# WangHelin1997/SSR-Speech

Measured on AMD Instinct MI355X. Metric: codec-tokens/sec/GPU (AR decode) + RTF for 10 s TTS, English 830M, higher is better.
Workload: dtype f32; 1 GPU; English-830M-shape zero-shot TTS decode, cfg_stride=5, top_k=40/top_p=0.8 sampling, batch=1 (2 CFG rows) per GPU; L=130 phonemes, 160-frame prompt (demo/5895_34622_000026_000002.wav, first 3.2 s, wmencodec codes), context 304..324; utterances_per_gpu=1, rows=2, graph=True, steps_completed=25, pair_launches=True

## Files before the change

ssr-speech_amd/csrc/gemv.hip:

```cpp
#include <stdlib.h>
#include "common.h"

namespace {

struct GemvK {
  ssrhip_gemv_args a;
  int nslice;
  int slice_len;
  int nch;
  int groups_x;
  int hd;
  int seg_shift;
  int rows_max;
  long long* prof;
  int rows_per, rows_rem;
};


long long* g_gemv_prof = nullptr;
constexpr int PRO_LN_REGS = 3;
constexpr int MAXCH = 8;
constexpr int MAX_IT = 8;

constexpr int NJ = 4;
// ... 699 lines not shown
  for (int j = 0; j < NUW; ++j) {
    float4 (&wj)[4] = w[j % DEPTH];
    float acc[B][2];
#pragma unroll
    for (int b = 0; b < B; ++b) acc[b][0] = acc[b][1] = 0.f;
#pragma unroll
    for (int i = 0; i < 4; ++i) {
#pragma unroll
      for (int b = 0; b < B; ++b) acc[b][i & 1] = dot4(wj[i], xr[b][i], acc[b][i & 1]);
      if (j + DEPTH < NUW) {
        __builtin_amdgcn_sched_barrier(0);
        wj[i] = ld_nt(Wg + (size_t)((wave + SEG_NW * (j + DEPTH)) >> sh) * K + i * 256);
        __builtin_amdgcn_sched_barrier(0);
      }
    }
    float mine = 0.f;
#pragma unroll
    for (int b = 0; b < B; ++b) {
      const float sum = wave_sum(acc[b][0] + acc[b][1]);
      if (lane == b) mine = sum;
    }
    if (lane < B) part[(wave + SEG_NW * j) * B + lane] = mine;
  }
  __syncthreads();
  if (t < nrows * B) {
    float v = 0.f;
    for (int s2 = 0; s2 < S; ++s2) v += part[(rfin * S + s2) * B + bfin];
    finalize(p, g, nfin, bfin, v, efin, kvb);
  }
}

constexpr int PAIR_D = 2048, PAIR_NE = 4, PAIR_TH = SEG_TH + 64 * PAIR_NE, PAIR_GRAN = 2 * PAIR_D, PAIR_PF = 3, PAIR_DEPTH = 4, PAIR_NUWA = 8;
constexpr int PAIR_SPINS = 4000000;
constexpr long long PAIR_WAIT_TICKS = 100000000;
struct PairK {
  GemvK a, b;
  unsigned long long* gran;
  unsigned long long* gran_next;
  int* gave_up;
};
typedef float pair_v4f __attribute__((ext_vector_type(4)));
__device__ __forceinline__ void pair_sweep8(const unsigned long long* p, pair_v4f (&g)[8]) {
  asm volatile(
      "global_load_dwordx4 %0, %8, off sc1\n\tglobal_load_dwordx4 %1, %8, off offset:1024 sc1\n\t"
      "global_load_dwordx4 %2, %8, off offset:2048 sc1\n\tglobal_load_dwordx4 %3, %8, off offset:3072 sc1\n\t"
      "global_load_dwordx4 %4, %9, off sc1\n\tglobal_load_dwordx4 %5, %9, off offset:1024 sc1\n\t"
      "global_load_dwordx4 %6, %9, off offset:2048 sc1\n\tglobal_load_dwordx4 %7, %9, off offset:3072 sc1\n\t"
      "s_waitcnt vmcnt(0)"
      : "=&v"(g[0]), "=&v"(g[1]), "=&v"(g[2]), "=&v"(g[3]), "=&v"(g[4]), "=&v"(g[5]), "=&v"(g[6]), "=&v"(g[7])
      : "v"(p), "v"(p + 512)
      : "memory");
}

template <int NUWB, int EARLY = 0, int PFX = PAIR_PF>
__device__ __forceinline__ void pair_stream_b(const PairK& p, int t, int lane, int wave, float4 (&xr)[2][4], float4 (&w)[PAIR_DEPTH][4],
                                              const RowEpi& efinB, float* partB, float* aux, const float* xs, const size_t* kvoff) {
  constexpr int B = 2, DEPTH = PAIR_DEPTH, PF = PFX, SB = 2, SHB = 1, RB = NUWB * SEG_NW / SB;
  static_assert(PFX >= EARLY && PFX <= PAIR_DEPTH, "units requested at (1b) start behind the early ones and fit the ring");
  static_assert(EARLY == 0 || EARLY == 2, "ring slots 2 and 3 are the ones the merge form's A phase leaves free");
  const ssrhip_gemv_args& bb = p.b.a;
  const int rB0 = (int)blockIdx.x * RB, segB = wave & (SB - 1);
  const int bfin = t % B, rfinB = min(t / B, RB - 1), nfinB = rB0 + rfinB;
  const float* WgB = bb.W + (size_t)rB0 * bb.K + segB * SEG + lane * 4;
  __syncthreads();
#pragma unroll
  for (int j = EARLY; j < PF; ++j)
#pragma unroll
    for (int i = 0; i < 4; ++i) w[(j + EARLY) % DEPTH][i] = ld_nt(WgB + (size_t)((wave + SEG_NW * j) >> SHB) * bb.K + i * 256);
  __syncthreads();
#pragma unroll
  for (int b = 0; b < B; ++b)
#pragma unroll
    for (int i = 0; i < 4; ++i) xr[b][i] = *reinterpret_cast<const float4*>(xs + b * PAIR_D + segB * SEG + (i * 64 + lane) * 4);
#pragma unroll
  for (int j = PF; j < DEPTH; ++j)
#pragma unroll
    for (int i = 0; i < 4; ++i) w[(j + EARLY) % DEPTH][i] = ld_nt(WgB + (size_t)((wave + SEG_NW * j) >> SHB) * bb.K + i * 256);
  {
    float m[B], q[B];
#pragma unroll
    for (int b = 0; b < B; ++b) {
      float s0 = 0.f;
#pragma unroll
      for (int i = 0; i < 4; ++i) s0 += (xr[b][i].x + xr[b][i].y) + (xr[b][i].z + xr[b][i].w);
      m[b] = wave_sum(s0) * (1.0f / SEG);
      float q0 = 0.f;
#pragma unroll
      for (int i = 0; i < 4; ++i) {
        const float dx = xr[b][i].x - m[b], dy = xr[b][i].y - m[b], dz = xr[b][i].z - m[b], dw = xr[b][i].w - m[b];
        q0 += (dx * dx + dy * dy) + (dz * dz + dw * dw);
      }
      q[b] = wave_sum(q0);
      if (wave < SB && lane == 0) { aux[(wave * B + b) * 2] = m[b]; aux[(wave * B + b) * 2 + 1] = q[b]; }
    }
    __syncthreads();
#pragma unroll
    for (int b = 0; b < B; ++b) {
      float mean = 0.f, M2 = 0.f, dev = 0.f;
      for (int s2 = 0; s2 < SB; ++s2) mean += aux[(s2 * B + b) * 2];
      mean /= (float)SB;
      for (int s2 = 0; s2 < SB; ++s2) { const float dm = aux[(s2 * B + b) * 2] - mean; M2 += aux[(s2 * B + b) * 2 + 1]; dev = fmaf(dm, dm, dev); }
      const float var = (M2 + (float)SEG * dev) / (float)bb.K;
      const float rstd = 1.0f / sqrtf(var + bb.ln_eps);
#pragma unroll
      for (int i = 0; i < 4; ++i)
        xr[b][i] = make_float4((xr[b][i].x - mean) * rstd, (xr[b][i].y - mean) * rstd, (xr[b][i].z - mean) * rstd, (xr[b][i].w - mean) * rstd);
    }
  }
#pragma unroll
  for (int j = 0; j < NUWB; ++j) {
    float4 (&wj)[4] = w[(j + EARLY) % DEPTH];
    float acc[B][2];
#pragma unroll
    for (int b = 0; b < B; ++b) acc[b][0] = acc[b][1] = 0.f;
#pragma unroll
    for (int i = 0; i < 4; ++i) {
#pragma unroll
      for (int b = 0; b < B; ++b) acc[b][i & 1] = dot4(wj[i], xr[b][i], acc[b][i & 1]);
      if (j + DEPTH < NUWB) {
        __builtin_amdgcn_sched_barrier(0);
        wj[i] = ld_nt(WgB + (size_t)((wave + SEG_NW * (j + DEPTH)) >> SHB) * bb.K + i * 256);
        __builtin_amdgcn_sched_barrier(0);
      }
    }
    float mine = 0.f;
#pragma unroll
    for (int b = 0; b < B; ++b) {
      const float sum = wave_sum(acc[b][0] + acc[b][1]);
      if (lane == b) mine = sum;
    }
    if (lane < B) partB[(wave + SEG_NW * j) * B + lane] = mine;
  }
  __syncthreads();
  if (t < RB * B) {
    float v = 0.f;
    for (int s2 = 0; s2 < SB; ++s2) v += partB[(rfinB * SB + s2) * B + bfin];
    float* kvb[2] = {bb.kv.pool + kvoff[bfin * 2], bb.kv.pool + kvoff[bfin * 2 + 1]};
    finalize(p.b, 0, nfinB, bfin, v, efinB, kvb);
  }
}

template <int SA, int NPRE>
__device__ __forceinline__ void pair_edge_role(const PairK& p, int e, int lane, const float* partA, float* xs, size_t* kvoff) {
  constexpr int B = 2, RA = 8;
  const ssrhip_gemv_args& a = p.a.a;
  const ssrhip_gemv_args& bb = p.b.a;
  const int rA0 = (int)blockIdx.x * RA;
  RowEpi efinA = {0.f, 0.f};
  if (e == 0 && lane < RA * B) {
    efinA.bias = a.bias ? a.bias[rA0 + (lane >> 1)] : 0.f;
    efinA.resid = a.y[(size_t)(lane & 1) * a.y_stride + rA0 + (lane >> 1)];
    p.gran_next[(size_t)blockIdx.x * (RA * B) + lane] = 0ull;
  }
  if (bb.epi == SSRHIP_EPI_QKV_APPEND && e == 1 && lane < B) {
    const int pos = bb.kv_pos[lane];
    const int page = bb.kv.table[(size_t)lane * bb.kv.max_pages + (pos / SSRHIP_PAGE)];
    const size_t k0 = ((((size_t)page * bb.kv.n_layer + bb.layer) * 2 + 0) * bb.kv.n_head) * SSRHIP_PAGE + (pos % SSRHIP_PAGE);
    const size_t v0 = ((((size_t)page * bb.kv.n_layer + bb.layer) * 2 + 1) * bb.kv.n_head) * SSRHIP_PAGE + (pos % SSRHIP_PAGE);
    kvoff[lane * 2 + 0] = k0 * bb.kv.head_dim;
    kvoff[lane * 2 + 1] = v0 * bb.kv.head_dim;
  }
#pragma unroll
  for (int i = 0; i < NPRE; ++i) __syncthreads();
  __syncthreads();
  if (e == 0 && lane < RA * B) {
    const int r = lane >> 1, b = lane & 1, n = rA0 + r;
    float v = 0.f;
    for (int s2 = 0; s2 < SA; ++s2) v += partA[(r * SA + s2) * B + b];
    v += efinA.bias;
    const float out = efinA.resid + v;
    a.y[(size_t)b * a.y_stride + n] = out;
    const unsigned long long gval = ((unsigned long long)1u << 32) | (unsigned long long)__float_as_uint(out);
    __hip_atomic_store(p.gran + (size_t)n * 2 + b, gval, __ATOMIC_RELAXED, __HIP_MEMORY_SCOPE_AGENT);
  }
  __syncthreads();
  pair_v4f g[8];
  bool done = false;
  const int max_spins = (*p.gave_up != 0) ? 64 : PAIR_SPINS;
  const long long t_begin = wall_clock64();
  for (int spin = 0; spin < max_spins && !done; ++spin) {
    bool all = true;
    pair_sweep8(p.gran + (size_t)e * 1024 + lane * 2, g);
#pragma unroll
    for (int i = 0; i < 8; ++i) {
      all = all && (__float_as_uint(g[i][1]) == 1u) && (__float_as_uint(g[i][3]) == 1u);
      const int gi = e * 1024 + (i >> 2) * 512 + (i & 3) * 128 + lane * 2;
      xs[(gi >> 1)] = g[i][0];
      xs[PAIR_D + (gi >> 1)] = g[i][2];
    }
    done = __all(all);
    if (!done) {
      __builtin_amdgcn_s_sleep(2);
// ... 32 lines not shown
    float4 w[DEPTH][4];
#pragma unroll
    for (int j = 0; j < DEPTH; ++j)
#pragma unroll
      for (int i = 0; i < 4; ++i) w[j][i] = ld_nt(WgA + (size_t)((wave + SEG_NW * j) >> SHA) * a.K + i * 256);
#pragma unroll
    for (int j = 0; j < NUWA; ++j) {
      float4 (&wj)[4] = w[j % DEPTH];
      float acc[B][2];
#pragma unroll
      for (int b = 0; b < B; ++b) acc[b][0] = acc[b][1] = 0.f;
#pragma unroll
      for (int i = 0; i < 4; ++i) {
#pragma unroll
        for (int b = 0; b < B; ++b) acc[b][i & 1] = dot4(wj[i], xr[b][i], acc[b][i & 1]);
        if (j + DEPTH < NUWA) {
          __builtin_amdgcn_sched_barrier(0);
          wj[i] = ld_nt(WgA + (size_t)((wave + SEG_NW * (j + DEPTH)) >> SHA) * a.K + i * 256);
          __builtin_amdgcn_sched_barrier(0);
        }
      }
      float mine = 0.f;
#pragma unroll
      for (int b = 0; b < B; ++b) {
        const float sum = wave_sum(acc[b][0] + acc[b][1]);
        if (lane == b) mine = sum;
      }
      if (lane < B) partA[(wave + SEG_NW * j) * B + lane] = mine;
    }
    __syncthreads();
    pair_stream_b<NUWB>(p, t, lane, wave, xr, w, efinB, partB, aux, xs, kvoff);
  } else {
    pair_edge_role<SA, 0>(p, wave - SEG_NW, lane, partA, xs, kvoff);
  }
}

template <int NUWB, int EARLY = 0, int PFX = PAIR_PF>
__global__ __launch_bounds__(PAIR_TH, 2) void gemv_pair_merge_kernel(const PairK p) {
  constexpr int B = 2, DEPTH = PAIR_DEPTH, SEG_CS = SegCS<B>::v;
  constexpr int RA = 8, SA = 2, SHA = 1;
  constexpr int RB = NUWB * SEG_NW / 2;
  extern __shared__ __attribute__((aligned(16))) float wtab[];
  __shared__ float partA[RA * SA * B];
  __shared__ float partB[RB * 2 * B];
  __shared__ float aux[2 * B * 2];
  __shared__ __attribute__((aligned(16))) float xs[B * PAIR_D];
  __shared__ size_t kvoff[B * 2];
  const ssrhip_gemv_args& a = p.a.a;
  const ssrhip_gemv_args& bb = p.b.a;
  const int t = threadIdx.x, lane = t & 63, wave = __builtin_amdgcn_readfirstlane(t >> 6);
  if (wave >= SEG_NW) {
    pair_edge_role<SA, 2>(p, wave - SEG_NW, lane, partA, xs, kvoff);
  } else {
    const int K = a.K, rA0 = (int)blockIdx.x * RA, seg = wave & (SA - 1);
    const float* WgA = a.W + (size_t)rA0 * K + seg * SEG + lane * 4;
    RowEpi efinB = {0.f, 0.f};
    efinB.bias = bb.bias ? bb.bias[(int)blockIdx.x * RB + min(t / B, RB - 1)] : 0.f;
    const int hd = p.a.hd, H = K / hd, MS = a.max_splits;
    float4 co[B][SEG_CS];
    float2 cml[SEG_CS];
    int ns[B];
#pragma unroll
    for (int b = 0; b < B; ++b) ns[b] = (a.row_len[b] + SSRHIP_PAGE - 1) / SSRHIP_PAGE;
    {
      const int tt = t % (B * H);
      const float* ml = a.part_ml + (size_t)tt * MS * 2;
#pragma unroll
      for (int i = 0; i < SEG_CS; ++i) cml[i] = *reinterpret_cast<const float2*>(ml + 2 * min(i, MS - 1));
      const int e = t * 4, h = e / hd, d = e % hd;
#pragma unroll
      for (int b = 0; b < B; ++b) {
        const float* po = a.part_o + (((size_t)b * H + h) * MS) * hd + d;
#pragma unroll
        for (int s2 = 0; s2 < SEG_CS; ++s2) co[b][s2] = ld4(po + (size_t)min(s2, MS - 1) * hd);
      }
    }
    float4 w[DEPTH][4];
#pragma unroll
    for (int j = 0; j < 2; ++j)
#pragma unroll
      for (int i = 0; i < 4; ++i) w[j][i] = ld_nt(WgA + (size_t)((wave + SEG_NW * j) >> SHA) * K + i * 256);
    if constexpr (EARLY == 2) {
      const float* WgB = bb.W + (size_t)((int)blockIdx.x * RB) * bb.K + (wave & 1) * SEG + lane * 4;
#pragma unroll
      for (int j = 0; j < 2; ++j)
#pragma unroll
        for (int i = 0; i < 4; ++i) w[2 + j][i] = ld_nt(WgB + (size_t)((wave + SEG_NW * j) >> 1) * bb.K + i * 256);
    }
    {
      const int tt = t % (B * H);
      const bool keep = t < B * H;
      const int n = ns[tt / H];
      const float* ml = a.part_ml + (size_t)tt * MS * 2;
      float M = -INFINITY;
#pragma unroll
      for (int i = 0; i < SEG_CS; ++i)
        if (i < n) M = fmaxf(M, cml[i].x);
      for (int s2 = SEG_CS; s2 < n; ++s2) M = fmaxf(M, ld2_late(ml + 2 * s2).x);
      float den = 0.f;
#pragma unroll
      for (int i = 0; i < SEG_CS; ++i)
        if (i < n) den = fmaf(expf(cml[i].x - M), cml[i].y, den);
      for (int s2 = SEG_CS; s2 < n; ++s2) { const float2 v = ld2_late(ml + 2 * s2); den = fmaf(expf(v.x - M), v.y, den); }
      const float inv = 1.0f / den;
#pragma unroll
      for (int i = 0; i < SEG_CS; ++i)
        if (keep && i < n) wtab[tt * MS + i] = expf(cml[i].x - M) * inv;
      for (int s2 = SEG_CS; s2 < n; ++s2) { const float wv = expf(ld2_late(ml + 2 * s2).x - M) * inv; if (keep) wtab[tt * MS + s2] = wv; }
    }
    __syncthreads();
    {
      const int e = t * 4, h = e / hd, d = e % hd;
#pragma unroll
      for (int b = 0; b < B; ++b) {
        const float* wt = wtab + (b * H + h) * MS;
        float4 acc = make_float4(0.f, 0.f, 0.f, 0.f);
#pragma unroll
        for (int s2 = 0; s2 < SEG_CS; ++s2) {
          const bool in = s2 < ns[b];
          const float ws = in ? wt[s2] : 0.f;
          acc.x = fmaf(ws, in ? co[b][s2].x : 0.f, acc.x);
          acc.y = fmaf(ws, in ? co[b][s2].y : 0.f, acc.y);
          acc.z = fmaf(ws, in ? co[b][s2].z : 0.f, acc.z);
          acc.w = fmaf(ws, in ? co[b][s2].w : 0.f, acc.w);
        }
        const float* po = a.part_o + (((size_t)b * H + h) * MS) * hd + d;
        for (int s2 = SEG_CS; s2 < ns[b]; ++s2) {
          const float ws = wt[s2];
          const float4 o = ld4_late(po + (size_t)s2 * hd);
          acc.x = fmaf(ws, o.x, acc.x);
          acc.y = fmaf(ws, o.y, acc.y);
          acc.z = fmaf(ws, o.z, acc.z);
          acc.w = fmaf(ws, o.w, acc.w);
        }
        *reinterpret_cast<float4*>(xs + b * K + e) = acc;
      }
    }
    __syncthreads();
    float4 xr[B][4];
#pragma unroll
    for (int b = 0; b < B; ++b)
#pragma unroll
      for (int i = 0; i < 4; ++i) xr[b][i] = *reinterpret_cast<const float4*>(xs + b * K + seg * SEG + (i * 64 + lane) * 4);
#pragma unroll
    for (int j = 0; j < 2; ++j) {
      float acc[B][2];
#pragma unroll
      for (int b = 0; b < B; ++b) acc[b][0] = acc[b][1] = 0.f;
#pragma unroll
      for (int i = 0; i < 4; ++i)
#pragma unroll
        for (int b = 0; b < B; ++b) acc[b][i & 1] = dot4(w[j][i], xr[b][i], acc[b][i & 1]);
      float mine = 0.f;
#pragma unroll
      for (int b = 0; b < B; ++b) {
        const float sum = wave_sum(acc[b][0] + acc[b][1]);
        if (lane == b) mine = sum;
      }
      if (lane < B) partA[(wave + SEG_NW * j) * B + lane] = mine;
    }
    __syncthreads();
    pair_stream_b<NUWB, EARLY, PFX>(p, t, lane, wave, xr, w, efinB, partB, aux, xs, kvoff);
  }
}

int g_seg_mode = -1;

template <int B>
bool try_seg(const ssrhip_gemv_args* a, int num_cu, hipStream_t s) {
  if (a->K % SEG != 0) return false;
  const int S = a->K / SEG;
  if (S != 1 && S != 2 && S != 4 && S != 8) return false;
  if (a->pro == SSRHIP_PRO_LAYERNORM && a->ln_w != nullptr) return false;
  const int H = a->kv.head_dim > 0 ? a->K / a->kv.head_dim : 0;
  if (a->pro == SSRHIP_PRO_ATTN_COMBINE && (a->K != 2048 || a->max_splits < 1 || a->groups != 1 || B * H > SEG_TH || a->kv.head_dim % 4 != 0)) return false;
  int G = (2 * num_cu) / a->groups;
  if (a->pro == SSRHIP_PRO_ATTN_COMBINE && !getenv("SSRHIP_GEMV_SEG_COMBINE_2")) G = num_cu;
  if (G > a->N) G = a->N;
  if (G < 1) G = 1;
  const int rows_max = (a->N + G - 1) / G;
  if (rows_max * B > SEG_TH) return false;
  GemvK p;
  p.a = *a;
  p.nslice = S;
  p.slice_len = SEG;
  p.nch = 4;
  p.seg_shift = (S == 1) ? 0 : (S == 2) ? 1 : (S == 4) ? 2 : 3;
  p.rows_max = rows_max;
  p.rows_per = a->N / G;
  p.rows_rem = a->N % G;
  p.prof = g_gemv_prof;
  p.groups_x = G;
  p.hd = (a->kv.head_dim > 0) ? a->kv.head_dim : 1;
  size_t smem = (size_t)rows_max * S * B * sizeof(float);
  if (a->pro == SSRHIP_PRO_LAYERNORM) smem += (size_t)S * B * 2 * sizeof(float);
  if (a->pro == SSRHIP_PRO_ATTN_COMBINE) smem += ((size_t)B * a->K + (size_t)B * H * a->max_splits) * sizeof(float);
  smem = (smem + 15) / 16 * 16;
  int segu_depth = 4;
  if (const char* e = getenv("SSRHIP_GEMV_SEGU")) { segu_depth = atoi(e); if (segu_depth != 0 && segu_depth != 2) segu_depth = 4; }
  if constexpr (B == 2) {
    const int G1 = num_cu / a->groups;
    if (segu_depth && a->pro != SSRHIP_PRO_ATTN_COMBINE && G1 >= 1 && a->N % G1 == 0 && ((a->N / G1) * S) % SEG_NW == 0) {
      const int nuw = (a->N / G1) * S / SEG_NW;
      if (nuw == 4 || nuw == 6 || nuw == 8) {
        p.rows_max = p.rows_per = a->N / G1;
        p.rows_rem = 0;
        p.groups_x = G1;
        size_t sm = (size_t)p.rows_per * S * B * sizeof(float) + (size_t)S * B * 2 * sizeof(float);
        sm = (sm + 15) / 16 * 16;
        const dim3 g1(G1, a->groups);
#define SEGU_LAUNCH(PRO_, NUW_)                                                                                                       \
        do {                                                                                                                           \
          if (segu_depth == 2) hipLaunchKernelGGL((gemv_segu_kernel<B, PRO_, NUW_, 2>), g1, dim3(SEG_TH), sm, s, p);                    \
          else hipLaunchKernelGGL((gemv_segu_kernel<B, PRO_, NUW_, 4>), g1, dim3(SEG_TH), sm, s, p);                                    \
        } while (0)
        if (a->pro == SSRHIP_PRO_LAYERNORM) {
          if (nuw == 4) SEGU_LAUNCH(SSRHIP_PRO_LAYERNORM, 4); else if (nuw == 6) SEGU_LAUNCH(SSRHIP_PRO_LAYERNORM, 6); else SEGU_LAUNCH(SSRHIP_PRO_LAYERNORM, 8);
        } else {
// ... 14 lines not shown
      if constexpr (B <= 2) { if (two) { hipLaunchKernelGGL((gemv_seg_kernel<B, SSRHIP_PRO_LAYERNORM, true>), grid, dim3(SEG_TH), smem, s, p); break; } }
      hipLaunchKernelGGL((gemv_seg_kernel<B, SSRHIP_PRO_LAYERNORM, false>), grid, dim3(SEG_TH), smem, s, p);
      break;
    case SSRHIP_PRO_ATTN_COMBINE:
      if constexpr (B <= 2) { if (two) { hipLaunchKernelGGL((gemv_seg_kernel<B, SSRHIP_PRO_ATTN_COMBINE, true>), grid, dim3(SEG_TH), smem, s, p); break; } }
      hipLaunchKernelGGL((gemv_seg_kernel<B, SSRHIP_PRO_ATTN_COMBINE, false>), grid, dim3(SEG_TH), smem, s, p);
      break;
    default:
      if constexpr (B <= 2) { if (two) { hipLaunchKernelGGL((gemv_seg_kernel<B, SSRHIP_PRO_NONE, true>), grid, dim3(SEG_TH), smem, s, p); break; } }
      hipLaunchKernelGGL((gemv_seg_kernel<B, SSRHIP_PRO_NONE, false>), grid, dim3(SEG_TH), smem, s, p);
      break;
  }
  return true;
}

int g_num_cu = 0;
int g_blocks_per_cu = 3;

}

int ssrhip_gemv_mfma_launch(const ssrhip_gemv_args* a, hipStream_t s);
int ssrhip_gemv_mfma32_launch(const ssrhip_gemv_args* a, hipStream_t s);

#ifdef SSR_GEMV_PROFILE
extern "C" void ssrhip_debug_gemv_prof(void* dev_ptr) { g_gemv_prof = (long long*)dev_ptr; }
#endif

static thread_local char g_pair_why[200] = "";
const char* ssrhip_gemv_pair_why() { return g_pair_why; }

static const char* pair_device_refusal(int num_cu) {
  static const char* verdict = nullptr;
  static bool asked = false;
  if (asked) return verdict;
  asked = true;
  static char buf[200];
  if (num_cu < 256) { snprintf(buf, sizeof(buf), "the device reports %d CUs (a pair launch needs its 256 workgroups resident together)", num_cu); return verdict = buf; }
  for (const char* name : {"ROC_GLOBAL_CU_MASK", "HSA_CU_MASK", "HSA_CU_MASK_SKIP_INIT"}) {
    const char* e = getenv(name);
    if (e && e[0]) { snprintf(buf, sizeof(buf), "%s is set: fewer CUs than the device reports may be usable", name); return verdict = buf; }
  }
  int nb[4] = {0, 0, 0, 0};
  hipError_t e0 = hipOccupancyMaxActiveBlocksPerMultiprocessor(&nb[0], gemv_pair_kernel<4>, PAIR_TH, 0);
  hipError_t e1 = hipOccupancyMaxActiveBlocksPerMultiprocessor(&nb[1], gemv_pair_kernel<6>, PAIR_TH, 0);
  hipError_t e2 = hipOccupancyMaxActiveBlocksPerMultiprocessor(&nb[2], gemv_pair_kernel<8>, PAIR_TH, 0);
  hipError_t e3 = hipOccupancyMaxActiveBlocksPerMultiprocessor(&nb[3], gemv_pair_merge_kernel<8, 2>, PAIR_TH, 16 * 1024);
  if (e0 != hipSuccess || e1 != hipSuccess || e2 != hipSuccess || e3 != hipSuccess || nb[0] < 1 || nb[1] < 1 || nb[2] < 1 || nb[3] < 1) {
    snprintf(buf, sizeof(buf), "the occupancy calculator places %d / %d / %d / %d workgroups of the pair kernels on a CU (need >= 1 each)", nb[0], nb[1], nb[2], nb[3]);
    return verdict = buf;
  }
  return verdict = nullptr;
}

static int pair_nuwb(const ssrhip_gemv_args* a, const ssrhip_gemv_args* b, int num_cu, bool* merge) {
  *merge = false;
  auto no = [](const char* why) { snprintf(g_pair_why, sizeof(g_pair_why), "%s", why); return 0; };
  int mode = 2;
  if (const char* e = getenv("SSRHIP_GEMV_PAIR")) mode = (e[0] == '0') ? 0 : (e[0] == '1') ? 1 : 2;
  if (mode == 0) return no("SSRHIP_GEMV_PAIR=0");
  if (const char* why = pair_device_refusal(num_cu)) return no(why);
  if (a->B != 2 || b->B != 2 || a->groups != 1 || b->groups != 1) return no("not a 2-row, single-group launch");
  if (a->x_tiled || a->y_tiled || a->w_tiled || b->x_tiled || b->y_tiled || b->w_tiled) return no("tiled layouts");
  if (a->act != SSRHIP_ACT_NONE || a->epi != SSRHIP_EPI_RESIDUAL || a->N != PAIR_D || !a->y || !a->W) return no("the first launch is not a residual GEMV with N = 2048 (the pair kernels are built for d_model 2048)");
  if (a->pro == SSRHIP_PRO_NONE) {
    if (a->K != 8192 || !a->x) return no("FFN2 form needs K = 8192");
  } else if (a->pro == SSRHIP_PRO_ATTN_COMBINE) {
    if (mode < 2) return no("SSRHIP_GEMV_PAIR=1: the merge form is off");
    const int hd = a->kv.head_dim;
    if (a->K != 2048 || !a->part_o || !a->part_ml || !a->row_len || a->max_splits < 1 || hd <= 0 || hd % 4 != 0 || a->K % hd != 0 || 2 * (a->K / hd) > SEG_TH) return no("merge form needs K = 2048 and split-KV partials");
    if ((size_t)2 * (a->K / hd) * a->max_splits * sizeof(float) > 16 * 1024) return no("merge weights exceed 16 KB of LDS (context too long for the merge form)");
    *merge = true;
  } else {
    return no("the first launch has a LayerNorm prologue");
  }
  if (b->pro != SSRHIP_PRO_LAYERNORM || b->ln_w || b->ln_b || b->K != PAIR_D || b->x != a->y || b->x_stride != a->y_stride || !b->W || !b->y) return no("the second launch is not LayerNorm (folded) + Linear on the first one's output");
  if (b->epi != SSRHIP_EPI_STORE && b->epi != SSRHIP_EPI_QKV_APPEND) return no("second launch: epilogue");
  if (b->epi == SSRHIP_EPI_QKV_APPEND && !(b->N == 3 * b->K && b->kv.pool && b->kv.table && b->kv_pos && b->kv.head_dim > 0)) return no("second launch: QKV append without a cache");
  if (b->N % 256 != 0) return no("second launch: N not a multiple of 256");
  const int nuwb = (b->N / 256) * 2 / SEG_NW;
  if ((b->N / 256) * 2 % SEG_NW != 0 || (nuwb != 4 && nuwb != 6 && nuwb != 8)) return no("second launch: N not in {4096, 6144, 8192}");
  if (*merge && nuwb != 8) return no("the merge form is instantiated for FFN1 only");
  g_pair_why[0] = 0;
  return nuwb;
}

static void ensure_num_cu() {
  if (g_num_cu == 0) {
    int dev = 0, cu = 0;
    if (hipGetDevice(&dev) == hipSuccess && hipDeviceGetAttribute(&cu, hipDeviceAttributeMultiprocessorCount, dev) == hipSuccess && cu > 0) g_num_cu = cu;
    else g_num_cu = 256;
    if (const char* e = getenv("SSRHIP_GEMV_BLOCKS_PER_CU")) { const int v = atoi(e); if (v >= 1 && v <= 3) g_blocks_per_cu = v; }
  }
}

extern "C" int ssrhip_pair_buffer(int32_t i, int32_t n) {
  if (n < 2 || i < 0 || i >= n) return -1;
  return (i == n - 1 && n % 3 == 1) ? 1 : i % 3;
}

extern "C" int ssrhip_gemv_pair_applicable(const ssrhip_gemv_args* a, const ssrhip_gemv_args* b) {
  if (!a || !b) return 0;
  ensure_num_cu();
  bool merge;
  return pair_nuwb(a, b, g_num_cu, &merge) != 0;
}

extern "C" int ssrhip_gemv_pair(const ssrhip_gemv_args* a, const ssrhip_gemv_args* b, void* ws, int32_t buf, int32_t buf_next, ssrhip_stream_t stream) {
  SSR_REQUIRE(a && b && ws, "ssrhip_gemv_pair: null argument");
  SSR_REQUIRE(buf >= 0 && buf < 3 && buf_next >= 0 && buf_next < 3 && buf != buf_next, "ssrhip_gemv_pair: granule buffers %d -> %d (0..2, different)", buf, buf_next);
  ensure_num_cu();
  bool merge = false;
  const int nuwb = pair_nuwb(a, b, g_num_cu, &merge);
  if (!nuwb) return 1;
  PairK p;
  auto fill = [](GemvK& k, const ssrhip_gemv_args* g, int S) {
    k.a = *g; k.nslice = S; k.slice_len = SEG; k.nch = 4; k.groups_x = 256; k.hd = (g->kv.head_dim > 0) ? g->kv.head_dim : 1;
    k.seg_shift = (S == 8) ? 3 : 1; k.rows_max = k.rows_per = g->N / 256; k.rows_rem = 0; k.prof = nullptr;
  };
  fill(p.a, a, merge ? 2 : 8);
  fill(p.b, b, 2);
  unsigned long long* gran = (unsigned long long*)ws;
  p.gran = gran + (size_t)buf * PAIR_GRAN;
  p.gran_next = gran + (size_t)buf_next * PAIR_GRAN;
  p.gave_up = (int*)(gran + 3 * (size_t)PAIR_GRAN);
  hipStream_t s = (hipStream_t)stream;
  if (merge) {
    const size_t sm = ((size_t)2 * (a->K / a->kv.head_dim) * a->max_splits * sizeof(float) + 15) / 16 * 16;
    const char* ee = getenv("SSRHIP_GEMV_PAIR_EARLY");
    if (ee && ee[0] == '0') hipLaunchKernelGGL((gemv_pair_merge_kernel<8, 0>), dim3(256), dim3(PAIR_TH), sm, s, p);
    else hipLaunchKernelGGL((gemv_pair_merge_kernel<8, 2>), dim3(256), dim3(PAIR_TH), sm, s, p);
  } else if (nuwb == 4) hipLaunchKernelGGL((gemv_pair_kernel<4>), dim3(256), dim3(PAIR_TH), 0, s, p);
  else if (nuwb == 6) hipLaunchKernelGGL((gemv_pair_kernel<6>), dim3(256), dim3(PAIR_TH), 0, s, p);
  else hipLaunchKernelGGL((gemv_pair_kernel<8>), dim3(256), dim3(PAIR_TH), 0, s, p);
  SSR_LAUNCH_CHECK();
  return 0;
}

extern "C" int ssrhip_gemv_pair_status(const void* ws, ssrhip_stream_t stream) {
  SSR_REQUIRE(ws, "ssrhip_gemv_pair_status: null workspace");
  int flag = 0;
  if (hipStreamSynchronize((hipStream_t)stream) != hipSuccess) { ssrhip_set_error("ssrhip_gemv_pair_status: stream synchronize failed"); return -1; }
  if (hipMemcpy(&flag, (const char*)ws + 3 * (size_t)PAIR_GRAN * 8, sizeof(int), hipMemcpyDeviceToHost) != hipSuccess) {
    ssrhip_set_error("ssrhip_gemv_pair_status: copy failed");
    return -1;
  }
  if (flag) {
    if (hipMemset(const_cast<void*>(ws), 0, SSRHIP_PAIR_WS_BYTES) != hipSuccess) { ssrhip_set_error("ssrhip_gemv_pair_status: re-zeroing the workspace failed"); return -1; }
  }
  return flag ? 1 : 0;
}

extern "C" int ssrhip_gemv(const ssrhip_gemv_args* a, ssrhip_stream_t stream) {
  SSR_REQUIRE(a && a->W && a->y, "ssrhip_gemv: null argument");
  SSR_REQUIRE(a->N > 0 && a->groups >= 1 && a->K > 0, "ssrhip_gemv: bad N/K/groups");
  if (a->B > 16) return ssrhip_gemv_mfma32_launch(a, (hipStream_t)stream);
  if (a->B > 4) return ssrhip_gemv_mfma_launch(a, (hipStream_t)stream);
  SSR_REQUIRE(a->B == 1 || a->B == 2 || a->B == 4, "ssrhip_gemv: B=%d not in {1,2,4} or 5..32", a->B);
  SSR_REQUIRE(!a->x_tiled && !a->y_tiled && !a->w_tiled, "ssrhip_gemv: the tiled activation / weight layouts are for 5..32 rows only");
  SSR_REQUIRE(a->pro != SSRHIP_PRO_ATTN_COMBINE || (a->kv.head_dim > 0 && a->K <= 2048 && a->B * (a->K / a->kv.head_dim) <= 256), "ssrhip_gemv: combine prologue needs K <= 2048 and B*H <= 256");
  SSR_REQUIRE(a->K > 0 && a->K % 4 == 0 && a->K <= 8192, "ssrhip_gemv: K=%d must be a multiple of 4, <= 8192", a->K);
  SSR_REQUIRE(a->N > 0 && a->groups >= 1, "ssrhip_gemv: bad N/groups");
  ensure_num_cu();
  if (a->pro != SSRHIP_PRO_NONE) {
    SSR_REQUIRE(a->groups == 1 || a->pro == SSRHIP_PRO_LAYERNORM, "ssrhip_gemv: combine prologue needs groups==1");
    if (a->pro == SSRHIP_PRO_LAYERNORM) SSR_REQUIRE(a->x && ((a->ln_w && a->ln_b) || (!a->ln_w && !a->ln_b)), "ssrhip_gemv: LayerNorm prologue needs x and either both or none of ln_w/ln_b");
    if (a->pro == SSRHIP_PRO_ATTN_COMBINE) {
      SSR_REQUIRE(a->part_o && a->part_ml && a->row_len && a->kv.head_dim > 0 && a->K % a->kv.head_dim == 0 && a->kv.head_dim % 4 == 0,
                  "ssrhip_gemv: combine prologue needs part_o, part_ml, row_len, kv.head_dim");
    }
  } else {
    SSR_REQUIRE(a->x, "ssrhip_gemv: x is null");
  }
  if (a->epi == SSRHIP_EPI_QKV_APPEND) {
    SSR_REQUIRE(a->N == 3 * a->K && a->groups == 1 && a->kv.pool && a->kv.table && a->kv_pos && a->kv.head_dim > 0,
                "ssrhip_gemv: QKV epilogue needs N==3K and a kv cache");
  }
  if (g_seg_mode < 0) { const char* e = getenv("SSRHIP_GEMV_SEG"); g_seg_mode = (e && e[0] == '0') ? 0 : 1; }
  if (g_seg_mode) {
    bool done = false;
    switch (a->B) {
      case 1: done = try_seg<1>(a, g_num_cu, (hipStream_t)stream); break;
      case 2: done = try_seg<2>(a, g_num_cu, (hipStream_t)stream); break;
// ... 54 lines not shown
```

Measured before the change: 5351 codec-tokens/s.

## Add LDS ring-buffer merge pair kernel with dedicated DMA loader waves

Adds a ring_merge_kernel variant of the merged attention-out plus QKV pair GEMV. Two extra loader waves use global_load_lds to stream second-GEMV weight units into an LDS ring while the compute waves run the first GEMV and the gather waves wait on cross-block granules. This is meant to hide the second GEMV's weight fetch latency behind the grid-wide handoff. It is on by default with a 2-slot ring, so it uses much more LDS and extra waves, which may lower occupancy or make it fall back to the register form when the merge weights do not fit. Optional profiling timestamps and lab variants are compiled out by default.

```diff
diff --git a/ssr-speech_amd/csrc/gemv.hip b/ssr-speech_amd/csrc/gemv.hip
--- a/ssr-speech_amd/csrc/gemv.hip
+++ b/ssr-speech_amd/csrc/gemv.hip
@@ -775,6 +775,11 @@
       : "memory");
 }
 
+#ifdef SSR_GEMV_PROFILE
+#define PSTAMP(i) do { if (p.a.prof && threadIdx.x == 0) p.a.prof[(size_t)blockIdx.x * 8 + (i)] = wall_clock64(); } while (0)
+#else
+#define PSTAMP(i) do { } while (0)
+#endif
 template <int NUWB, int EARLY = 0, int PFX = PAIR_PF>
 __device__ __forceinline__ void pair_stream_b(const PairK& p, int t, int lane, int wave, float4 (&xr)[2][4], float4 (&w)[PAIR_DEPTH][4],
                                               const RowEpi& efinB, float* partB, float* aux, const float* xs, const size_t* kvoff) {
@@ -785,12 +790,15 @@
   const int rB0 = (int)blockIdx.x * RB, segB = wave & (SB - 1);
   const int bfin = t % B, rfinB = min(t / B, RB - 1), nfinB = rB0 + rfinB;
   const float* WgB = bb.W + (size_t)rB0 * bb.K + segB * SEG + lane * 4;
-  __syncthreads();
+  PSTAMP(2);
+  __syncthreads();
+  PSTAMP(3);
 #pragma unroll
   for (int j = EARLY; j < PF; ++j)
 #pragma unroll
     for (int i = 0; i < 4; ++i) w[(j + EARLY) % DEPTH][i] = ld_nt(WgB + (size_t)((wave + SEG_NW * j) >> SHB) * bb.K + i * 256);
   __syncthreads();
+  PSTAMP(4);
 #pragma unroll
   for (int b = 0; b < B; ++b)
 #pragma unroll
@@ -853,7 +861,9 @@
       if (lane == b) mine = sum;
     }
     if (lane < B) partB[(wave + SEG_NW * j) * B + lane] = mine;
-  }
+    if (j == 0) PSTAMP(5);
+  }
+  PSTAMP(6);
   __syncthreads();
   if (t < RB * B) {
     float v = 0.f;
@@ -861,6 +871,7 @@
     float* kvb[2] = {bb.kv.pool + kvoff[bfin * 2], bb.kv.pool + kvoff[bfin * 2 + 1]};
     finalize(p.b, 0, nfinB, bfin, v, efinB, kvb);
   }
+  PSTAMP(7);
 }
 
 template <int SA, int NPRE>
@@ -999,6 +1010,7 @@
   if (wave >= SEG_NW) {
     pair_edge_role<SA, 2>(p, wave - SEG_NW, lane, partA, xs, kvoff);
   } else {
+    PSTAMP(0);
     const int K = a.K, rA0 = (int)blockIdx.x * RA, seg = wave & (SA - 1);
     const float* WgA = a.W + (size_t)rA0 * K + seg * SEG + lane * 4;
     RowEpi efinB = {0.f, 0.f};
@@ -1084,6 +1096,7 @@
       }
     }
     __syncthreads();
+    PSTAMP(1);
     float4 xr[B][4];
 #pragma unroll
     for (int b = 0; b < B; ++b)
@@ -1111,6 +1124,372 @@
   }
 }
 
+constexpr int RING_SLOT = 8192;
+constexpr int RING_FILL = 16;
+typedef __attribute__((address_space(3))) void* ring_lds_ptr_t;
+
+__device__ __forceinline__ void ring_dma_kib(const float* gsrc, unsigned lds_dst) {
+  unsigned keep;
+  asm volatile("s_mov_b32 %0, m0\n\ts_mov_b32 m0, %2\n\ts_nop 0\n\tglobal_load_lds_dwordx4 %1, off nt\n\ts_mov_b32 m0, %0"
+               : "=&s"(keep) : "v"(gsrc), "s"(lds_dst) : "memory");
+}
+template <int N>
+__device__ __forceinline__ void ring_wait_vm() { asm volatile("s_waitcnt vmcnt(%0)" :: "n"(N) : "memory"); }
+
+__device__ __forceinline__ void ring_fill(const float* WgL, int K, unsigned ring_addr, int L, int s) {
+#pragma unroll
+  for (int ww = 0; ww < 4; ++ww) {
+    const int w = 4 * L + ww;
+    const float* src = WgL + (size_t)((w + SEG_NW * (2 + s)) >> 1) * K + (w & 1) * SEG;
+#pragma unroll
+    for (int i = 0; i < 4; ++i) ring_dma_kib(src + i * 256, __builtin_amdgcn_readfirstlane(ring_addr + (unsigned)(s * RING_SLOT + w * 1024 + i * 256) * 4u));
+  }
+}
+
+__device__ __forceinline__ void ring_sweep16(const unsigned long long* p, pair_v4f (&g)[16]) {
+  asm volatile(
+      "global_load_dwordx4 %0, %16, off sc1\n\tglobal_load_dwordx4 %1, %16, off offset:1024 sc1\n\t"
+      "global_load_dwordx4 %2, %16, off offset:2048 sc1\n\tglobal_load_dwordx4 %3, %16, off offset:3072 sc1\n\t"
+      "global_load_dwordx4 %4, %17, off sc1\n\tglobal_load_dwordx4 %5, %17, off offset:1024 sc1\n\t"
+      "global_load_dwordx4 %6, %17, off offset:2048 sc1\n\tglobal_load_dwordx4 %7, %17, off offset:3072 sc1\n\t"
+      "global_load_dwordx4 %8, %18, off sc1\n\tglobal_load_dwordx4 %9, %18, off offset:1024 sc1\n\t"
+      "global_load_dwordx4 %10, %18, off offset:2048 sc1\n\tglobal_load_dwordx4 %11, %18, off offset:3072 sc1\n\t"
+      "global_load_dwordx4 %12, %19, off sc1\n\tglobal_load_dwordx4 %13, %19, off offset:1024 sc1\n\t"
+      "global_load_dwordx4 %14, %19, off offset:2048 sc1\n\tglobal_load_dwordx4 %15, %19, off offset:3072 sc1\n\t"
+      "s_waitcnt vmcnt(0)"
+      : "=&v"(g[0]), "=&v"(g[1]), "=&v"(g[2]), "=&v"(g[3]), "=&v"(g[4]), "=&v"(g[5]), "=&v"(g[6]), "=&v"(g[7]),
+        "=&v"(g[8]), "=&v"(g[9]), "=&v"(g[10]), "=&v"(g[11]), "=&v"(g[12]), "=&v"(g[13]), "=&v"(g[14]), "=&v"(g[15])
+      : "v"(p), "v"(p + 512), "v"(p + 1024), "v"(p + 1536)
+      : "memory");
+}
+
+template <bool PFIRST>
+__device__ __forceinline__ void ring_gather_role(const PairK& p, int e, int lane, const float* partA, float* xs, size_t* kvoff) {
+  constexpr int B = 2, RA = 8, SA = 2;
+  const ssrhip_gemv_args& a = p.a.a;
+  const ssrhip_gemv_args& bb = p.b.a;
+  const int rA0 = (int)blockIdx.x * RA;
+  RowEpi efinA = {0.f, 0.f};
+  if (e == 0 && lane < RA * B) {
+    efinA.bias = a.bias ? a.bias[rA0 + (lane >> 1)] : 0.f;
+    efinA.resid = a.y[(size_t)(lane & 1) * a.y_stride + rA0 + (lane >> 1)];
+    p.gran_next[(size_t)blockIdx.x * (RA * B) + lane] = 0ull;
+  }
+  if (bb.epi == SSRHIP_EPI_QKV_APPEND && e == 1 && lane < B) {
+    const int pos = bb.kv_pos[lane];
+    const int page = bb.kv.table[(size_t)lane * bb.kv.max_pages + (pos / SSRHIP_PAGE)];
+    const size_t k0 = ((((size_t)page * bb.kv.n_layer + bb.layer) * 2 + 0) * bb.kv.n_head) * SSRHIP_PAGE + (pos % SSRHIP_PAGE);
+    const size_t v0 = ((((size_t)page * bb.kv.n_layer + bb.layer) * 2 + 1) * bb.kv.n_head) * SSRHIP_PAGE + (pos % SSRHIP_PAGE);
+    kvoff[lane * 2 + 0] = k0 * bb.kv.head_dim;
+    kvoff[lane * 2 + 1] = v0 * bb.kv.head_dim;
+  }
+  if constexpr (PFIRST) __syncthreads();
+  __syncthreads();
+  __syncthreads();
+  __syncthreads();
+  if (e == 0 && lane < RA * B) {
+    const int r = lane >> 1, b = lane & 1, n = rA0 + r;
+    float v = 0.f;
+    for (int s2 = 0; s2 < SA; ++s2) v += partA[(r * SA + s2) * B + b];
+    v += efinA.bias;
+    const float out = efinA.resid + v;
+    a.y[(size_t)b * a.y_stride + n] = out;
+    const unsigned long long gval = ((unsigned long long)1u << 32) | (unsigned long long)__float_as_uint(out);
+    __hip_atomic_store(p.gran + (size_t)n * 2 + b, gval, __ATOMIC_RELAXED, __HIP_MEMORY_SCOPE_AGENT);
+  }
+  __syncthreads();
+  pair_v4f g[16];
+  bool done = false;
+  const int max_spins = (*p.gave_up != 0) ? 64 : PAIR_SPINS;
+  const long long t_begin = wall_clock64();
+  for (int spin = 0; spin < max_spins && !done; ++spin) {
+    bool all = true;
+    ring_sweep16(p.gran + (size_t)e * 2048 + lane * 2, g);
+#pragma unroll
+    for (int i = 0; i < 16; ++i) {
+      all = all && (__float_as_uint(g[i][1]) == 1u) && (__float_as_uint(g[i][3]) == 1u);
+      const int gi = e * 2048 + (i >> 2) * 512 + (i & 3) * 128 + lane * 2;
+      xs[(gi >> 1)] = g[i][0];
+      xs[PAIR_D + (gi >> 1)] = g[i][2];
+    }
+    done = __all(all);
+    if (!done) {
+      __builtin_amdgcn_s_sleep(2);
+      if ((spin & 255) == 255 && wall_clock64() - t_begin > PAIR_WAIT_TICKS) break;
+    }
+  }
+  if (!done && lane == 0) *p.gave_up = 1;
+  __syncthreads();
+  __syncthreads();
+  __syncthreads();
+}
+
+template <int NR, int P, bool FULLW, bool PFIRST>
+__device__ __forceinline__ void ring_load_role(const PairK& p, int L, int lane, const float* ring, volatile int* full) {
+  static_assert(NR >= 1 && NR <= 4 && P >= 1 && P < NR && RING_FILL * P <= 63, "fills in flight: fewer than the ring has, countable by vmcnt");
+  const ssrhip_gemv_args& bb = p.b.a;
+  const unsigned ring_addr = (unsigned)(uintptr_t)(ring_lds_ptr_t)ring;
+  const float* WgL = bb.W + (size_t)((int)blockIdx.x * 32) * bb.K + lane * 4;
+  const int K = bb.K;
+  if (FULLW && lane == 0) full[L] = 0;
+  if constexpr (PFIRST) __builtin_amdgcn_s_barrier();
+#pragma unroll
+  for (int f = 0; f < P; ++f) ring_fill(WgL, K, ring_addr, L, f);
+  asm volatile("s_waitcnt lgkmcnt(0)" ::: "memory");
+  __builtin_amdgcn_s_barrier();
+  __builtin_amdgcn_s_barrier();
+  __builtin_amdgcn_s_barrier();
+  __builtin_amdgcn_s_barrier();
+#pragma unroll
+  for (int f = P; f < NR; ++f) {
+    ring_fill(WgL, K, ring_addr, L, f);
+    ring_wait_vm<RING_FILL * P>();
+  }
+  __builtin_amdgcn_s_barrier();
+  if constexpr (!FULLW) ring_wait_vm<0>();
+  __builtin_amdgcn_s_barrier();
+  if constexpr (FULLW) {
+    ring_wait_vm<0>();
+    if (lane == 0) full[L] = 1;
+    asm volatile("s_waitcnt lgkmcnt(0)" ::: "memory");
+  }
+  __builtin_amdgcn_s_barrier();
+}
+
+template <int NR, int P, bool FULLW, bool PFIRST>
+__global__ __launch_bounds__(PAIR_TH, 2) void ring_merge_kernel(const PairK p) {
+  constexpr int B = 2, DEPTH = PAIR_DEPTH, SEG_CS = SegCS<B>::v, NUWB = 8;
+  constexpr int RA = 8, SA = 2, SHA = 1;
+  constexpr int RB = NUWB * SEG_NW / 2, SB = 2, SHB = 1;
+  constexpr int MID = 4 - NR;
+  extern __shared__ __attribute__((aligned(16))) float ring[];
+  float* const wtab = ring + NR * RING_SLOT;
+  __shared__ float partA[RA * SA * B];
+  __shared__ float partB[RB * 2 * B];
+  __shared__ float aux[2 * B * 2];
+  __shared__ __attribute__((aligned(16))) float xs[B * PAIR_D];
+  __shared__ size_t kvoff[B * 2];
+  __shared__ volatile int full[2];
+  const ssrhip_gemv_args& a = p.a.a;
+  const ssrhip_gemv_args& bb = p.b.a;
+  const int t = threadIdx.x, lane = t & 63, wave = __builtin_amdgcn_readfirstlane(t >> 6);
+#ifdef SSR_PAIR_RING_NANFILL
+  for (int i = t; i < NR * RING_SLOT; i += PAIR_TH) ring[i] = __builtin_nanf("");
+  __syncthreads();
+#endif
+  if (wave >= SEG_NW + 2) {
+    ring_load_role<NR, P, FULLW, PFIRST>(p, wave - SEG_NW - 2, lane, ring, full);
+  } else if (wave >= SEG_NW) {
+    ring_gather_role<PFIRST>(p, wave - SEG_NW, lane, partA, xs, kvoff);
+  } else {
+    PSTAMP(0);
+    const int K = a.K, rA0 = (int)blockIdx.x * RA, seg = wave & (SA - 1);
+    const float* WgA = a.W + (size_t)rA0 * K + seg * SEG + lane * 4;
+    RowEpi efinB = {0.f, 0.f};
+    efinB.bias = bb.bias ? bb.bias[(int)blockIdx.x * RB + min(t / B, RB - 1)] : 0.f;
+    const int hd = p.a.hd, H = K / hd, MS = a.max_splits;
+    float4 co[B][SEG_CS];
+    float2 cml[SEG_CS];
+    int ns[B];
+#pragma unroll
+    for (int b = 0; b < B; ++b) ns[b] = (a.row_len[b] + SSRHIP_PAGE - 1) / SSRHIP_PAGE;
+    {
+      const int tt = t % (B * H);
+      const float* ml = a.part_ml + (size_t)tt * MS * 2;
+#pragma unroll
+      for (int i = 0; i < SEG_CS; ++i) cml[i] = *reinterpret_cast<const float2*>(ml + 2 * min(i, MS - 1));
+      const int e = t * 4, h = e / hd, d = e % hd;
+#pragma unroll
+      for (int b = 0; b < B; ++b) {
+        const float* po = a.part_o + (((size_t)b * H + h) * MS) * hd + d;
+#pragma unroll
+        for (int s2 = 0; s2 < SEG_CS; ++s2) co[b][s2] = ld4(po + (size_t)min(s2, MS - 1) * hd);
+      }
+    }
+    if constexpr (PFIRST) {
+      __builtin_amdgcn_sched_barrier(0);
+      __builtin_amdgcn_s_barrier();
+      __builtin_amdgcn_sched_barrier(0);
+    }
+    float4 w[DEPTH][4];
+#pragma unroll
+    for (int j = 0; j < 2; ++j)
+#pragma unroll
+      for (int i = 0; i < 4; ++i) w[j][i] = ld_nt(WgA + (size_t)((wave + SEG_NW * j) >> SHA) * K + i * 256);
+    const int segB = wave & (SB - 1);
+    const float* WgB = bb.W + (size_t)((int)blockIdx.x * RB) * bb.K + segB * SEG + lane * 4;
+#pragma unroll
+    for (int j = 0; j < 2; ++j)
+#pragma unroll
+      for (int i = 0; i < 4; ++i) w[2 + j][i] = ld_nt(WgB + (size_t)((wave + SEG_NW * j) >> SHB) * bb.K + i * 256);
+    {
+      const int tt = t % (B * H);
+      const bool keep = t < B * H;
+      const int n = ns[tt / H];
+      const float* ml = a.part_ml + (size_t)tt * MS * 2;
+      float M = -INFINITY;
+#pragma unroll
+      for (int i = 0; i < SEG_CS; ++i)
+        if (i < n) M = fmaxf(M, cml[i].x);
+      for (int s2 = SEG_CS; s2 < n; ++s2) M = fmaxf(M, ld2_late(ml + 2 * s2).x);
+      float den = 0.f;
+#pragma unroll
+      for (int i = 0; i < SEG_CS; ++i)
+        if (i < n) den = fmaf(expf(cml[i].x - M), cml[i].y, den);
+      for (int s2 = SEG_CS; s2 < n; ++s2) { const float2 v = ld2_late(ml + 2 * s2); den = fmaf(expf(v.x - M), v.y, den); }
+      const float inv = 1.0f / den;
+#pragma unroll
+      for (int i = 0; i < SEG_CS; ++i)
+        if (keep && i < n) wtab[tt * MS + i] = expf(cml[i].x - M) * inv;
+      for (int s2 = SEG_CS; s2 < n; ++s2) { const float wv = expf(ld2_late(ml + 2 * s2).x - M) * inv; if (keep) wtab[tt * MS + s2] = wv; }
+    }
+    __syncthreads();
+    {
+      const int e = t * 4, h = e / hd, d = e % hd;
+#pragma unroll
+      for (int b = 0; b < B; ++b) {
+        const float* wt = wtab + (b * H + h) * MS;
+        float4 acc = make_float4(0.f, 0.f, 0.f, 0.f);
+#pragma unroll
+        for (int s2 = 0; s2 < SEG_CS; ++s2) {
+          const bool in = s2 < ns[b];
+          const float ws = in ? wt[s2] : 0.f;
+          acc.x = fmaf(ws, in ? co[b][s2].x : 0.f, acc.x);
+          acc.y = fmaf(ws, in ? co[b][s2].y : 0.f, acc.y);
+          acc.z = fmaf(ws, in ? co[b][s2].z : 0.f, acc.z);
+          acc.w = fmaf(ws, in ? co[b][s2].w : 0.f, acc.w);
+        }
+        const float* po = a.part_o + (((size_t)b * H + h) * MS) * hd + d;
+        for (int s2 = SEG_CS; s2 < ns[b]; ++s2) {
+          const float ws = wt[s2];
+          const float4 o = ld4_late(po + (size_t)s2 * hd);
+          acc.x = fmaf(ws, o.x, acc.x);
+          acc.y = fmaf(ws, o.y, acc.y);
+          acc.z = fmaf(ws, o.z, acc.z);
+          acc.w = fmaf(ws, o.w, acc.w);
+        }
+        *reinterpret_cast<float4*>(xs + b * K + e) = acc;
+      }
+    }
+    __syncthreads();
+    PSTAMP(1);
+    float4 xr[B][4];
+#pragma unroll
+    for (int b = 0; b < B; ++b)
+#pragma unroll
+      for (int i = 0; i < 4; ++i) xr[b][i] = *reinterpret_cast<const float4*>(xs + b * K + seg * SEG + (i * 64 + lane) * 4);
+#pragma unroll
+    for (int j = 0; j < 2; ++j) {
+      float acc[B][2];
+#pragma unroll
+      for (int b = 0; b < B; ++b) acc[b][0] = acc[b][1] = 0.f;
+#pragma unroll
+      for (int i = 0; i < 4; ++i)
+#pragma unroll
+        for (int b = 0; b < B; ++b) acc[b][i & 1] = dot4(w[j][i], xr[b][i], acc[b][i & 1]);
+      float mine = 0.f;
+#pragma unroll
+      for (int b = 0; b < B; ++b) {
+        const float sum = wave_sum(acc[b][0] + acc[b][1]);
+        if (lane == b) mine = sum;
+      }
+      if (lane < B) partA[(wave + SEG_NW * j) * B + lane] = mine;
+    }
+    __syncthreads();
+    const int bfin = t % B, rfinB = min(t / B, RB - 1), nfinB = (int)blockIdx.x * RB + rfinB;
+    PSTAMP(2);
+    __syncthreads();
+    PSTAMP(3);
+#pragma unroll
+    for (int i = 0; i < 4; ++i) w[0][i] = ld_nt(WgB + (size_t)((wave + SEG_NW * 6) >> SHB) * bb.K + i * 256);
+    __syncthreads();
+    PSTAMP(4);
+#pragma unroll
+    for (int b = 0; b < B; ++b)
+#pragma unroll
+      for (int i = 0; i < 4; ++i) xr[b][i] = *reinterpret_cast<const float4*>(xs + b * PAIR_D + segB * SEG + (i * 64 + lane) * 4);
+#pragma unroll
+    for (int i = 0; i < 4; ++i) w[1][i] = ld_nt(WgB + (size_t)((wave + SEG_NW * 7) >> SHB) * bb.K + i * 256);
+    {
+      float m[B], q[B];
+#pragma unroll
+      for (int b = 0; b < B; ++b) {
+        float s0 = 0.f;
+#pragma unroll
+        for (int i = 0; i < 4; ++i) s0 += (xr[b][i].x + xr[b][i].y) + (xr[b][i].z + xr[b][i].w);
+        m[b] = wave_sum(s0) * (1.0f / SEG);
+        float q0 = 0.f;
+#pragma unroll
+        for (int i = 0; i < 4; ++i) {
+          const float dx = xr[b][i].x - m[b], dy = xr[b][i].y - m[b], dz = xr[b][i].z - m[b], dw = xr[b][i].w - m[b];
+          q0 += (dx * dx + dy * dy) + (dz * dz + dw * dw);
+        }
+        q[b] = wave_sum(q0);
+        if (wave < SB && lane == 0) { aux[(wave * B + b) * 2] = m[b]; aux[(wave * B + b) * 2 + 1] = q[b]; }
+      }
+      __syncthreads();
+#pragma unroll
+      for (int b = 0; b < B; ++b) {
+        float mean = 0.f, M2 = 0.f, dev = 0.f;
+        for (int s2 = 0; s2 < SB; ++s2) mean += aux[(s2 * B + b) * 2];
+        mean /= (float)SB;
+        for (int s2 = 0; s2 < SB; ++s2) { const float dm = aux[(s2 * B + b) * 2] - mean; M2 += aux[(s2 * B + b) * 2 + 1]; dev = fmaf(dm, dm, dev); }
+        const float var = (M2 + (float)SEG * dev) / (float)bb.K;
+        const float rstd = 1.0f / sqrtf(var + bb.ln_eps);
+#pragma unroll
+        for (int i = 0; i < 4; ++i)
+          xr[b][i] = make_float4((xr[b][i].x - mean) * rstd, (xr[b][i].y - mean) * rstd, (xr[b][i].z - mean) * rstd, (xr[b][i].w - mean) * rstd);
+      }
+    }
+#pragma unroll
+    for (int j = 0; j < NUWB; ++j) {
+      float4 wl[4];
+      if (j >= 2 && j < 2 + NR) {
+        if (FULLW && j == 2 + NR - P) {
+          const long long t_begin = wall_clock64();
+          int spin = 0;
+          while ((full[0] == 0 || full[1] == 0) && ++spin < PAIR_SPINS)
+            if ((spin & 255) == 255 && wall_clock64() - t_begin > PAIR_WAIT_TICKS) break;
+          if ((full[0] == 0 || full[1] == 0) && lane == 0) *p.gave_up = 1;
+          asm volatile("" ::: "memory");
+        }
+#pragma unroll
+        for (int i = 0; i < 4; ++i) wl[i] = *reinterpret_cast<const float4*>(ring + (j - 2) * RING_SLOT + wave * 1024 + (i * 64 + lane) * 4);
+      }
+      float4 (&wj)[4] = (j < 2) ? w[2 + j] : (j < 2 + NR) ? wl : (j < 6) ? w[2 + (j + 6 - NR) % 2] : w[j - 6];
+      float acc[B][2];
+#pragma unroll
+      for (int b = 0; b < B; ++b) acc[b][0] = acc[b][1] = 0.f;
+#pragma unroll
+      for (int i = 0; i < 4; ++i) {
+#pragma unroll
+        for (int b = 0; b < B; ++b) acc[b][i & 1] = dot4(wj[i], xr[b][i], acc[b][i & 1]);
+        if (j < MID) {
+          __builtin_amdgcn_sched_barrier(0);
+          wj[i] = ld_nt(WgB + (size_t)((wave + SEG_NW * (2 + NR + j)) >> SHB) * bb.K + i * 256);
+          __builtin_amdgcn_sched_barrier(0);
+        }
+      }
+      float mine = 0.f;
+#pragma unroll
+      for (int b = 0; b < B; ++b) {
+        const float sum = wave_sum(acc[b][0] + acc[b][1]);
+        if (lane == b) mine = sum;
+      }
+      if (lane < B) partB[(wave + SEG_NW * j) * B + lane] = mine;
+      if (j == 0) PSTAMP(5);
+    }
+    PSTAMP(6);
+    __syncthreads();
+    if (t < RB * B) {
+      float v = 0.f;
+      for (int s2 = 0; s2 < SB; ++s2) v += partB[(rfinB * SB + s2) * B + bfin];
+      float* kvb[2] = {bb.kv.pool + kvoff[bfin * 2], bb.kv.pool + kvoff[bfin * 2 + 1]};
+      finalize(p.b, 0, nfinB, bfin, v, efinB, kvb);
+    }
+    PSTAMP(7);
+  }
+}
 int g_seg_mode = -1;
 
 template <int B>
@@ -1231,6 +1610,74 @@
   return verdict = nullptr;
 }
 
+template <int NR, int P, bool FULLW, bool PFIRST>
+struct RingVariant { static int max_sm; };
+template <int NR, int P, bool FULLW, bool PFIRST> int RingVariant<NR, P, FULLW, PFIRST>::max_sm = -1;
+
+template <int NR, int P, bool FULLW, bool PFIRST = false>
+static void ring_setup_one() {
+  int& max_sm = RingVariant<NR, P, FULLW, PFIRST>::max_sm;
+  max_sm = -1;
+  const size_t ring_bytes = (size_t)NR * RING_SLOT * sizeof(float);
+  hipFuncAttributes fa;
+  if (hipFuncGetAttributes(&fa, reinterpret_cast<const void*>(&ring_merge_kernel<NR, P, FULLW, PFIRST>)) != hipSuccess) { (void)hipGetLastError(); return; }
+  const size_t room = 160 * 1024 - ((fa.sharedSizeBytes + 255) / 256 * 256);
+  const size_t dyn_max = ring_bytes + 16 * 1024 < room ? ring_bytes + 16 * 1024 : room;
+  if (hipFuncSetAttribute(reinterpret_cast<const void*>(&ring_merge_kernel<NR, P, FULLW, PFIRST>), hipFuncAttributeMaxDynamicSharedMemorySize, (int)dyn_max) != hipSuccess) {
+    (void)hipGetLastError();
+#ifdef SSR_PAIR_RING_LAB
+    fprintf(stderr, "ring_merge_kernel<%d, %d>: the LDS limit could not be raised to %zu B: the register form runs\n", NR, P, dyn_max);
+#endif
+    return;
+  }
+  for (int sm = (int)(dyn_max - ring_bytes) / 256 * 256; sm >= 0; sm -= 256) {
+    int nb = 0;
+    if (hipOccupancyMaxActiveBlocksPerMultiprocessor(&nb, ring_merge_kernel<NR, P, FULLW, PFIRST>, PAIR_TH, ring_bytes + (size_t)sm) != hipSuccess) { (void)hipGetLastError(); nb = 0; }
+    if (nb >= 1) { max_sm = sm; break; }
+  }
+#ifdef SSR_PAIR_RING_LAB
+  if (max_sm < 0) fprintf(stderr, "ring_merge_kernel<%d, %d>: no workgroup fits a CU: the register form runs\n", NR, P);
+#endif
+}
+static void ring_setup() {
+  static ssr_once_per_device once;
+  if (!once.need()) return;
+  ring_setup_one<2, 1, false>();
+#ifdef SSR_PAIR_RING_LAB
+  ring_setup_one<4, 1, false>(); ring_setup_one<4, 2, false>(); ring_setup_one<4, 1, true>(); ring_setup_one<3, 1, false>(); ring_setup_one<4, 3, false>();
+  ring_setup_one<4, 1, false, true>(); ring_setup_one<3, 2, false>(); ring_setup_one<2, 1, false, true>();
+#endif
+}
+template <int NR, int P, bool FULLW, bool PFIRST = false>
+static bool ring_try(const PairK& p, size_t sm, hipStream_t s) {
+  if ((long)sm > (long)RingVariant<NR, P, FULLW, PFIRST>::max_sm) {
+#ifdef SSR_PAIR_RING_LAB
+    fprintf(stderr, "ring_merge_kernel<%d, %d>: %zu B of merge weights do not fit behind the ring: the register form runs\n", NR, P, sm);
+#endif
+    return false;
+  }
+  hipLaunchKernelGGL((ring_merge_kernel<NR, P, FULLW, PFIRST>), dim3(256), dim3(PAIR_TH), (size_t)NR * RING_SLOT * sizeof(float) + sm, s, p);
+  return true;
+}
+static bool ring_launch(const PairK& p, size_t sm, hipStream_t s) {
+  const char* e = getenv("SSRHIP_GEMV_PAIR_RING");
+  if (e && e[0] == '0') return false;
+#ifdef SSR_PAIR_RING_LAB
+  switch ((e && e[0] >= '1' && e[0] <= '9') ? e[0] - '0' : 6) {
+    case 1: return ring_try<4, 1, false>(p, sm, s);
+    case 2: return ring_try<4, 2, false>(p, sm, s);
+    case 3: return ring_try<4, 1, true>(p, sm, s);
+    case 4: return ring_try<3, 1, false>(p, sm, s);
+    case 5: return ring_try<4, 3, false>(p, sm, s);
+    case 7: return ring_try<4, 1, false, true>(p, sm, s);
+    case 8: return ring_try<3, 2, false>(p, sm, s);
+    case 9: return ring_try<2, 1, false, true>(p, sm, s);
+    default: break;
+  }
+#endif
+  return ring_try<2, 1, false>(p, sm, s);
+}
+
 static int pair_nuwb(const ssrhip_gemv_args* a, const ssrhip_gemv_args* b, int num_cu, bool* merge) {
   *merge = false;
   auto no = [](const char* why) { snprintf(g_pair_why, sizeof(g_pair_why), "%s", why); return 0; };
@@ -1238,6 +1685,7 @@
   if (const char* e = getenv("SSRHIP_GEMV_PAIR")) mode = (e[0] == '0') ? 0 : (e[0] == '1') ? 1 : 2;
   if (mode == 0) return no("SSRHIP_GEMV_PAIR=0");
   if (const char* why = pair_device_refusal(num_cu)) return no(why);
+  ring_setup();
   if (a->B != 2 || b->B != 2 || a->groups != 1 || b->groups != 1) return no("not a 2-row, single-group launch");
   if (a->x_tiled || a->y_tiled || a->w_tiled || b->x_tiled || b->y_tiled || b->w_tiled) return no("tiled layouts");
   if (a->act != SSRHIP_ACT_NONE || a->epi != SSRHIP_EPI_RESIDUAL || a->N != PAIR_D || !a->y || !a->W) return no("the first launch is not a residual GEMV with N = 2048 (the pair kernels are built for d_model 2048)");
@@ -1297,6 +1745,9 @@
     k.seg_shift = (S == 8) ? 3 : 1; k.rows_max = k.rows_per = g->N / 256; k.rows_rem = 0; k.prof = nullptr;
   };
   fill(p.a, a, merge ? 2 : 8);
+#ifdef SSR_GEMV_PROFILE
+  if (merge) p.a.prof = g_gemv_prof;
+#endif
   fill(p.b, b, 2);
   unsigned long long* gran = (unsigned long long*)ws;
   p.gran = gran + (size_t)buf * PAIR_GRAN;
@@ -1306,7 +1757,9 @@
   if (merge) {
     const size_t sm = ((size_t)2 * (a->K / a->kv.head_dim) * a->max_splits * sizeof(float) + 15) / 16 * 16;
     const char* ee = getenv("SSRHIP_GEMV_PAIR_EARLY");
-    if (ee && ee[0] == '0') hipLaunchKernelGGL((gemv_pair_merge_kernel<8, 0>), dim3(256), dim3(PAIR_TH), sm, s, p);
+    const bool early = !(ee && ee[0] == '0');
+    if (early && ring_launch(p, sm, s)) { SSR_LAUNCH_CHECK(); return 0; }
+    if (!early) hipLaunchKernelGGL((gemv_pair_merge_kernel<8, 0>), dim3(256), dim3(PAIR_TH), sm, s, p);
     else hipLaunchKernelGGL((gemv_pair_merge_kernel<8, 2>), dim3(256), dim3(PAIR_TH), sm, s, p);
   } else if (nuwb == 4) hipLaunchKernelGGL((gemv_pair_kernel<4>), dim3(256), dim3(PAIR_TH), 0, s, p);
   else if (nuwb == 6) hipLaunchKernelGGL((gemv_pair_kernel<6>), dim3(256), dim3(PAIR_TH), 0, s, p);
```

Result: no change. 5334 codec-tokens/s (-0.3%).
